# xingchensong/TouchNet

Hardware: AMD Instinct MI355X
Metric: audio+text tokens/sec/node (packed seq, full train step) + step MFU (higher is better)
Workload: dtype bf16

## Files before the change

touchnet_amd/csrc/gemm_kernel.h:

```cpp
#pragma once

#include <stdlib.h>

#include <type_traits>
#include <utility>
#include <vector>

#include "common.h"

namespace tn {
namespace gemm {

constexpr int BM = 256, BN = 256;
constexpr int SLOT = 32768;
constexpr int LDS_BYTES = 5 * SLOT;
constexpr int NT = 512;
constexpr int MAXSEG = 3;

typedef __attribute__((address_space(3))) void* lds_ptr_t;
typedef __attribute__((ext_vector_type(2))) uint32_t u32x2_t;
typedef __attribute__((ext_vector_type(4))) uint32_t u32x4_t;

struct Seg {
  const bf16_t* A;
  const bf16_t* B;
  long long lda, ldb;
  int K;
  int pad_;
};

struct Grp {
  bf16_t* C;
  long long ldc;
  int M, N, nbm, nbn;
  int start;
  int stages;
};

struct Rec {
  Seg seg;
  Grp grp;
  bf16_t* bias_out;
};
typedef const __attribute__((address_space(4))) Rec* rec_ptr_t;
constexpr int MAXTAB = 1024;
constexpr int TABCHUNK = 32;

constexpr int EPI_PLAIN = 0, EPI_GROUPED = 1, EPI_SWIGLU_FWD = 2, EPI_SWIGLU_BWD = 3, EPI_BIASG = 4, EPI_ROPE = 5;
constexpr int EPI_GELU_FWD = 6, EPI_GELU_BWD = 7, EPI_TABLE = 8;

struct Params {
  Seg seg[MAXSEG];
  int nseg;
  int M, N;
  bf16_t* C;
  bf16_t* Ct;
  const bf16_t* bias;
  long long ldc, ldct;
  int accumulate;
  const bf16_t* addend;
  long long ldadd;
  int nbm, nbn;
  int stages;
  int splitk, kchunk;
  float* ws;
  int tile0, ntiles;
  int c_f32;
  Grp grp[MAXSEG];
  int ngrp;
  bf16_t* C2;
  bf16_t* C3;
  const bf16_t* E1;
  const bf16_t* E2;
  long long lde;
  bf16_t* bias_out;
  float* bias_ws;
  const bf16_t* rope_cos;
  const bf16_t* rope_sin;
  int rope_d;
  const Rec* table;
};

__device__ __forceinline__ int xcd_chunk(int bid, int total) {
  const int xcd = bid & 7, local = bid >> 3;
  const int q = total >> 3, r = total & 7;
  return (xcd < r ? xcd * (q + 1) : r * (q + 1) + (xcd - r) * q) + local;
}

__device__ __forceinline__ void panel_group(int vid, int nbm, int nbn, int& tm, int& tn) {
  constexpr int GM = 8;
  const int per_group = GM * nbn;
  const int g = vid / per_group, w = vid - g * per_group;
  const int gm = min(GM, nbm - g * GM);
  tm = g * GM + w % gm;
  tn = w / gm;
}

__device__ __forceinline__ void tile_of_block(int bid, int nbm, int nbn, int& tm, int& tn) {
  panel_group(xcd_chunk(bid, nbm * nbn), nbm, nbn, tm, tn);
}

typedef f32x16_t Acc[4][2];

constexpr int kPieceB[4] = {0, 2, 4, 6}, kPieceA[4] = {14, 18, 22, 26};
static_assert(kPieceB[3] < kPieceA[0], "every B piece is issued before the first A piece");

template <bool IS_A> constexpr int piece_at(int pos) {
  for (int i = 0; i < 4; ++i)
    if ((IS_A ? kPieceA[i] : kPieceB[i]) == pos) return i;
  return -1;
}
constexpr int early_piece_count() {
  int n = 0;
  for (int i = 0; i < 4; ++i) n += (kPieceB[i] < 8) + (kPieceA[i] < 8);
  return n;
}

template <bool KMAJ, bool M16 = false>
struct Stream {
  __amdgpu_buffer_rsrc_t rs;
  int soff;
  int step;
  int left;
  int seg;
  int ld2;
  int voff[4];

  __device__ __forceinline__ void set_voff(int wave, int lane) {
    if constexpr (!KMAJ) {
#pragma unroll
      for (int q = 0; q < 4; ++q) {
        const int row = wave * 32 + q * 8 + (lane >> 3);
        voff[q] = row * ld2 + (((lane & 7) ^ ((row >> 1) & 7)) << 4);
      }
    } else {
#pragma unroll
      for (int q = 0; q < 4; ++q) {
        const int k = wave * 8 + q * 2 + (lane >> 5);
        const int u = lane & 31;
        const int ch = M16 ? ((u & 3) ^ (((k >> 3) & 1) << 1)) : (u & 3);
        voff[q] = k * ld2 + ((((u >> 2) ^ (k & 3)) << 6) | (ch << 4));
      }
    }
  }

  __device__ __forceinline__ void open(const bf16_t* X, long long ld, int K, int R, int origin, int wave, int lane) {
    ld2 = (int)(ld * 2);
    if constexpr (!KMAJ) {
      const long long bytes = max((long long)(R - origin) * ld2, 0LL);
      rs = __builtin_amdgcn_make_buffer_rsrc((void*)(X + (long long)origin * ld), 0, (int)min(bytes, 0x7fffffffLL),
                                             0x00020000);
      step = 128;
    } else {
      const long long bytes = ((long long)(K - 1) * ld + (R - origin)) * 2;
      rs = __builtin_amdgcn_make_buffer_rsrc((void*)(X + origin), 0, (int)min(bytes, 0x7fffffffLL), 0x00020000);
      step = 64 * ld2;
    }
    set_voff(wave, lane);
    soff = 0;
    left = (K + 63) >> 6;
  }
  __device__ __forceinline__ void kill(const void* any) {
    rs = __builtin_amdgcn_make_buffer_rsrc((void*)any, 0, 0, 0x00020000);
    soff = 0;
    step = 0;
    left = 0x7fffffff;
  }
};

template <bool KMAJ, int NB>
struct Frags {
  bf16x8_t v[NB];
  u32x2_t h[KMAJ ? NB : 1][2];
};

template <int OFF>
__device__ __forceinline__ u32x2_t ds_tr16(uint32_t addr) {
  u32x2_t r;
  asm volatile("ds_read_b64_tr_b16 %0, %1 offset:%2" : "=v"(r) : "v"(addr), "n"(OFF));
  return r;
}

template <bool AK, bool BK, bool HAS_CT, bool SPLITK = false, bool OUT_F32 = false, int EPI = EPI_PLAIN>
struct Kernel {
  static_assert(EPI == EPI_PLAIN || EPI == EPI_GROUPED || EPI == EPI_BIASG || EPI == EPI_TABLE,
                "Kernel: plain / grouped / bias-gradient epilogues (the fused ones are Kernel16's)");
  static constexpr bool MULTI = EPI == EPI_GROUPED || EPI == EPI_TABLE;
  static constexpr bool BIASG = EPI == EPI_BIASG || EPI == EPI_TABLE;
  static_assert(!MULTI || (!HAS_CT && !SPLITK), "grouped launch: whole tiles, no transposed copy");
  static_assert(!BIASG || (AK && BK && !HAS_CT), "bias gradient: weight-gradient mode");
  struct Out {
    bf16_t* C;
    long long ldc;
    int M, N;
  };
  template <bool KMAJ, int NB>
  struct Reader {
    int x[4];
    __device__ __forceinline__ Reader(int lane, int row0 ) {
      const int l31 = lane & 31, hi = lane >> 5;
      if constexpr (!KMAJ) {
        const int f = (l31 >> 1) & 7;
#pragma unroll
        for (int q = 0; q < 4; ++q) x[q] = (row0 + l31) * 128 + (((2 * q + hi) ^ f) << 4);
      } else {
        const int s4 = lane & 15, j = s4 >> 2, w = s4 & 3, half = (lane >> 4) & 1;
#pragma unroll
        for (int b = 0; b < 4; ++b)
          x[b] = (8 * hi + j) * 512 + half * 32 + w * 8 + ((((row0 >> 5) + (b < NB ? b : 0)) ^ j) << 6);
      }
    }
    template <int Q, int B>
    __device__ __forceinline__ void read(const char* smem, int sbase, Frags<KMAJ, NB>& f) const {
      if constexpr (!KMAJ) {
        f.v[B] = __builtin_bit_cast(bf16x8_t, *reinterpret_cast<const u32x4_t*>(smem + sbase + x[Q] + B * 4096));
      } else {
        const uint32_t a = (uint32_t)(size_t)(lds_ptr_t)smem + (uint32_t)(sbase + x[B]);
        f.h[B][0] = ds_tr16<(16 * Q) * 512>(a);
        f.h[B][1] = ds_tr16<(16 * Q + 4) * 512>(a);
      }
    }
  };

  static __device__ __forceinline__ void wait_frags(Frags<AK, 4>& a, Frags<BK, 2>& b) {
    if constexpr (AK && BK) {
      asm volatile("s_waitcnt lgkmcnt(0)"
                   : "+v"(a.h[0][0]), "+v"(a.h[0][1]), "+v"(a.h[1][0]), "+v"(a.h[1][1]), "+v"(a.h[2][0]), "+v"(a.h[2][1]),
                     "+v"(a.h[3][0]), "+v"(a.h[3][1]), "+v"(b.h[0][0]), "+v"(b.h[0][1]), "+v"(b.h[1][0]), "+v"(b.h[1][1]));
    } else if constexpr (AK) {
      asm volatile("s_waitcnt lgkmcnt(0)"
                   : "+v"(a.h[0][0]), "+v"(a.h[0][1]), "+v"(a.h[1][0]), "+v"(a.h[1][1]), "+v"(a.h[2][0]), "+v"(a.h[2][1]),
                     "+v"(a.h[3][0]), "+v"(a.h[3][1]));
    } else if constexpr (BK) {
      asm volatile("s_waitcnt lgkmcnt(0)" : "+v"(b.h[0][0]), "+v"(b.h[0][1]), "+v"(b.h[1][0]), "+v"(b.h[1][1]));
    }
    if constexpr (AK) {
#pragma unroll
      for (int i = 0; i < 4; ++i) {
        const u32x4_t t = {a.h[i][0].x, a.h[i][0].y, a.h[i][1].x, a.h[i][1].y};
        a.v[i] = __builtin_bit_cast(bf16x8_t, t);
      }
    }
    if constexpr (BK) {
#pragma unroll
      for (int j = 0; j < 2; ++j) {
        const u32x4_t t = {b.h[j][0].x, b.h[j][0].y, b.h[j][1].x, b.h[j][1].y};
        b.v[j] = __builtin_bit_cast(bf16x8_t, t);
      }
    }
  }

  static __device__ __forceinline__ void run(const Params& p, char* smem) { body(p, smem); }

  static __device__ __forceinline__ void body(const Params& p, char* smem) {
    const int tid = threadIdx.x;
    int lane = tid & 63;
    const int wave = __builtin_amdgcn_readfirstlane(tid >> 6);
    const int wr = wave >> 2, wc = wave & 3;

    const int bid = blockIdx.x, G = gridDim.x;
    const int tiles = p.ntiles;
    const int mine = ((SPLITK ? tiles * p.splitk : tiles) - bid + G - 1) / G;
    const rec_ptr_t tab = (rec_ptr_t)p.table;
    auto seg_of = [&](int g) {
      if constexpr (EPI == EPI_TABLE) {
        Seg s;
        s.A = tab[g].seg.A;
        s.B = tab[g].seg.B;
        s.lda = tab[g].seg.lda;
        s.ldb = tab[g].seg.ldb;
        s.K = tab[g].seg.K;
        s.pad_ = 0;
        return s;
      } else {
        return p.seg[g];
      }
    };
    auto grp_of = [&](int g) {
      if constexpr (EPI == EPI_TABLE) {
        Grp r;
        r.C = tab[g].grp.C;
        r.ldc = tab[g].grp.ldc;
        r.M = tab[g].grp.M;
        r.N = tab[g].grp.N;
        r.nbm = tab[g].grp.nbm;
        r.nbn = tab[g].grp.nbn;
        r.start = tab[g].grp.start;
        r.stages = tab[g].grp.stages;
        return r;
      } else {
        return p.grp[g];
      }
    };
    auto origin_g = [&](int k, int& m0, int& n0, int& g) {
      int tm, tn, u = bid + k * G;
      if constexpr (SPLITK) u -= (u / tiles) * tiles;
      u += p.tile0;
      g = 0;
      if constexpr (EPI == EPI_TABLE) {
        u = xcd_chunk(u, tiles);
        int hi = p.ngrp - 1;
        while (g < hi) {
          const int mid = (g + hi + 1) >> 1;
          if (tab[mid].grp.start <= u) g = mid;
          else hi = mid - 1;
        }
      } else if constexpr (EPI == EPI_GROUPED) {
        if (p.ngrp > 1 && u >= p.grp[1].start) g = 1;
        if (p.ngrp > 2 && u >= p.grp[2].start) g = 2;
      }
      if constexpr (EPI == EPI_TABLE) {
        const Grp r = grp_of(g);
        panel_group(u - r.start, r.nbm, r.nbn, tm, tn);
      } else if constexpr (EPI == EPI_GROUPED) {
        const Grp r = grp_of(g);
        tile_of_block(u - r.start, r.nbm, r.nbn, tm, tn);
      } else {
        tile_of_block(u, p.nbm, p.nbn, tm, tn);
      }
      m0 = tm * BM;
      n0 = tn * BN;
    };
    auto origin = [&](int k, int& m0, int& n0) {
      int g;
      origin_g(k, m0, n0, g);
    };
    auto split_of = [&](int k) { return (bid + k * G) / tiles; };

    Stream<AK> sA;
    Stream<BK> sB;
    int ka = 0, kb = 0;
    auto open_a = [&](int s) {
      int m0, n0;
      origin(ka, m0, n0);
      if constexpr (SPLITK) {
        const int k0 = split_of(ka) * p.kchunk * 64, klen = min(p.seg[0].K - k0, p.kchunk * 64);
        if (klen > 0) sA.open(p.seg[0].A + (AK ? (long long)k0 * p.seg[0].lda : (long long)k0), p.seg[0].lda, klen, p.M,
                              m0, wave, lane);
        else sA.kill(p.C);
        sA.left = p.kchunk;
      } else if constexpr (MULTI) {
        int g;
        origin_g(ka, m0, n0, g);
        const Seg sg = seg_of(g);
        sA.open(sg.A, sg.lda, sg.K, grp_of(g).M, m0, wave, lane);
      } else {
        sA.open(p.seg[s].A, p.seg[s].lda, p.seg[s].K, p.M, m0, wave, lane);
      }
      sA.seg = s;
    };
    auto open_b = [&](int s) {
      int m0, n0;
      origin(kb, m0, n0);
      if constexpr (SPLITK) {
        const int k0 = split_of(kb) * p.kchunk * 64, klen = min(p.seg[0].K - k0, p.kchunk * 64);
        if (klen > 0) sB.open(p.seg[0].B + (BK ? (long long)k0 * p.seg[0].ldb : (long long)k0), p.seg[0].ldb, klen, p.N,
                              n0, wave, lane);
        else sB.kill(p.C);
        sB.left = p.kchunk;
      } else if constexpr (MULTI) {
        int g;
        origin_g(kb, m0, n0, g);
        const Seg sg = seg_of(g);
        sB.open(sg.B, sg.ldb, sg.K, grp_of(g).N, n0, wave, lane);
      } else {
        sB.open(p.seg[s].B, p.seg[s].ldb, p.seg[s].K, p.N, n0, wave, lane);
      }
      sB.seg = s;
    };
    auto adv_a = [&]() {
      sA.soff += sA.step;
      if (--sA.left == 0) {
        if (sA.seg + 1 < p.nseg) open_a(sA.seg + 1);
        else if (++ka < mine) open_a(0);
        else sA.kill(p.C);
      }
    };
    auto adv_b = [&]() {
      sB.soff += sB.step;
      if (--sB.left == 0) {
        if (sB.seg + 1 < p.nseg) open_b(sB.seg + 1);
        else if (++kb < mine) open_b(0);
        else sB.kill(p.C);
      }
    };
    auto piece_a = [&](int slot, int q) {
      __builtin_amdgcn_raw_ptr_buffer_load_lds(sA.rs, (lds_ptr_t)(smem + slot * SLOT + wave * 4096 + q * 1024), 16,
                                               sA.voff[q], sA.soff, 0, 0);
    };
    auto piece_b = [&](int slot, int q) {
      __builtin_amdgcn_raw_ptr_buffer_load_lds(sB.rs, (lds_ptr_t)(smem + slot * SLOT + wave * 4096 + q * 1024), 16,
                                               sB.voff[q], sB.soff, 0, 0);
    };
    open_a(0);
    open_b(0);

    Reader<AK, 4> ra(lane, wr * 128);
    Reader<BK, 2> rb(lane, wc * 64);

    Acc acc;
    auto zero_acc = [&]() {
#pragma unroll
      for (int i = 0; i < 4; ++i)
#pragma unroll
        for (int j = 0; j < 2; ++j)
#pragma unroll
          for (int r = 0; r < 16; ++r) acc[i][j][r] = 0.f;
    };
    zero_acc();

    Frags<AK, 4> ae, ao;
    Frags<BK, 2> be, bo;

#define TN_PIN() __builtin_amdgcn_sched_barrier(0)
    auto read_frag = [&](auto QC, auto FC, int sa, int sb, Frags<AK, 4>& a, Frags<BK, 2>& b) {
      constexpr int Q = decltype(QC)::value, F = decltype(FC)::value;
      if constexpr (F < 2) rb.template read<Q, F>(smem, sb * SLOT, b);
      else ra.template read<Q, F - 2>(smem, sa * SLOT, a);
    };
    auto read_all = [&](auto QC, int sa, int sb, Frags<AK, 4>& a, Frags<BK, 2>& b) {
      read_frag(QC, std::integral_constant<int, 0>{}, sa, sb, a, b);
      read_frag(QC, std::integral_constant<int, 1>{}, sa, sb, a, b);
      read_frag(QC, std::integral_constant<int, 2>{}, sa, sb, a, b);
      read_frag(QC, std::integral_constant<int, 3>{}, sa, sb, a, b);
      read_frag(QC, std::integral_constant<int, 4>{}, sa, sb, a, b);
      read_frag(QC, std::integral_constant<int, 5>{}, sa, sb, a, b);
    };
    auto mma = [&](const Frags<AK, 4>& a, const Frags<BK, 2>& b, int i, int j) {
      acc[i][j] = __builtin_amdgcn_mfma_f32_32x32x16_bf16(b.v[j], a.v[i], acc[i][j], 0, 0, 0);
    };

    float bsum = 0.f;
    bool bias_on = false;
    auto bias_accum = [&](const Frags<AK, 4>& a) {
      auto add = [&](const bf16x8_t& v) {
        const u32x4_t w = __builtin_bit_cast(u32x4_t, v);
        bsum += ((__uint_as_float(w.x << 16) + __uint_as_float(w.x & 0xffff0000u)) +
                 (__uint_as_float(w.y << 16) + __uint_as_float(w.y & 0xffff0000u))) +
                ((__uint_as_float(w.z << 16) + __uint_as_float(w.z & 0xffff0000u)) +
                 (__uint_as_float(w.w << 16) + __uint_as_float(w.w & 0xffff0000u)));
      };
      if (wc == 0) add(a.v[0]);
      else if (wc == 1) add(a.v[1]);
      else if (wc == 2) add(a.v[2]);
      else add(a.v[3]);
    };

    auto quarter = [&](auto NQC, auto P0C, const Frags<AK, 4>& ca, const Frags<BK, 2>& cb, Frags<AK, 4>& na,
                       Frags<BK, 2>& nb, int nsa, int nsb, int dst_b, int dst_a) {
      constexpr int P0 = decltype(P0C)::value;
      if constexpr (BIASG) {
        if (bias_on) bias_accum(ca);
        TN_PIN();
      }
      auto step = [&](auto MC) {
        constexpr int m = decltype(MC)::value;
        mma(ca, cb, m >> 1, m & 1);
        TN_PIN();
        if constexpr (m < 6) {
          read_frag(NQC, std::integral_constant<int, m>{}, nsa, nsb, na, nb);
          TN_PIN();
        }
        constexpr int pb = P0 < 0 ? -1 : piece_at<false>(P0 + m);
        constexpr int pa = P0 < 0 ? -1 : piece_at<true>(P0 + m);
        if constexpr (pb >= 0) {
          piece_b(dst_b, pb);
          if constexpr (pb == 3) adv_b();
          TN_PIN();
        }
        if constexpr (pa >= 0) {
          piece_a(dst_a, pa);
          if constexpr (pa == 3) adv_a();
          TN_PIN();
        }
      };
      step(std::integral_constant<int, 0>{});
      step(std::integral_constant<int, 1>{});
      step(std::integral_constant<int, 2>{});
      step(std::integral_constant<int, 3>{});
      step(std::integral_constant<int, 4>{});
      step(std::integral_constant<int, 5>{});
      step(std::integral_constant<int, 6>{});
      step(std::integral_constant<int, 7>{});
    };
    auto early_pieces = [&](int dst_b, int dst_a) {
      auto one = [&](auto MC) {
        constexpr int m = decltype(MC)::value;
        constexpr int pb = piece_at<false>(m), pa = piece_at<true>(m);
        if constexpr (pb >= 0) {
          piece_b(dst_b, pb);
          if constexpr (pb == 3) adv_b();
        }
        if constexpr (pa >= 0) {
          piece_a(dst_a, pa);
          if constexpr (pa == 3) adv_a();
        }
      };
      one(std::integral_constant<int, 0>{});
      one(std::integral_constant<int, 1>{});
      one(std::integral_constant<int, 2>{});
      one(std::integral_constant<int, 3>{});
      one(std::integral_constant<int, 4>{});
      one(std::integral_constant<int, 5>{});
      one(std::integral_constant<int, 6>{});
      one(std::integral_constant<int, 7>{});
    };
    auto next = [](int s, int d) { s += d; return s >= 5 ? s - 5 : s; };
    using I0 = std::integral_constant<int, 0>;
    using I1 = std::integral_constant<int, 1>;
    using I2 = std::integral_constant<int, 2>;
    using I3 = std::integral_constant<int, 3>;
    using NONE = std::integral_constant<int, -1>;

#pragma unroll
    for (int q = 0; q < 4; ++q) piece_a(0, q);
    adv_a();
#pragma unroll
    for (int q = 0; q < 4; ++q) piece_b(1, q);
    adv_b();
#pragma unroll
    for (int q = 0; q < 4; ++q) piece_a(2, q);
    adv_a();
    early_pieces(3, 4);
    asm volatile("s_waitcnt vmcnt(%0)" ::"n"(4 + early_piece_count()) : "memory");
    __builtin_amdgcn_s_barrier();
    int sa = 0, sb = 1;
    int pa = 4, pb = 3;

    auto trip = [&](auto LASTC) {
      constexpr bool LAST = decltype(LASTC)::value;
      const int sa1 = next(sa, 2), sb1 = next(sb, 2);
      __builtin_amdgcn_s_setprio(1);
      quarter(I1{}, std::integral_constant<int, 8>{}, ae, be, ao, bo, sa, sb, pb, pa);
      wait_frags(ao, bo);
      TN_PIN();
      quarter(I2{}, std::integral_constant<int, 16>{}, ao, bo, ae, be, sa, sb, pb, pa);
      wait_frags(ae, be);
      TN_PIN();
      quarter(I3{}, std::integral_constant<int, 24>{}, ae, be, ao, bo, sa, sb, pb, pa);
      __builtin_amdgcn_s_setprio(0);
      wait_frags(ao, bo);
      __builtin_amdgcn_s_waitcnt(0xc07f);
      asm volatile("s_waitcnt vmcnt(4)" ::: "memory");
      __builtin_amdgcn_s_barrier();
      __builtin_amdgcn_s_setprio(1);
      if constexpr (!LAST) {
        quarter(I0{}, I0{}, ao, bo, ae, be, sa1, sb1, sa, sb);
        __builtin_amdgcn_s_setprio(0);
        wait_frags(ae, be);
        TN_PIN();
      } else {
        if constexpr (BIASG) {
          if (bias_on) bias_accum(ao);
        }
#pragma unroll
        for (int m = 0; m < 8; ++m) mma(ao, bo, m >> 1, m & 1);
        __builtin_amdgcn_s_setprio(0);
      }
      pb = sa;
      pa = sb;
      sa = sa1;
      sb = sb1;
    };

    const int np_all = SPLITK ? p.kchunk : p.stages;
    for (int kc = 0; kc < mine; ++kc) {
      int np = np_all;
      if constexpr (BIASG) {
        int m0_, n0_, g_;
        origin_g(kc, m0_, n0_, g_);
        bias_on = n0_ == 0;
        if constexpr (EPI == EPI_TABLE) bias_on = bias_on && tab[g_].bias_out != nullptr;
        bsum = 0.f;
      }
      if constexpr (MULTI) {
        int m0_, n0_, g_;
        origin_g(kc, m0_, n0_, g_);
        np = grp_of(g_).stages;
      }
      read_all(I0{}, sa, sb, ae, be);
      wait_frags(ae, be);
      TN_PIN();
      for (int t = 1; t < np; ++t) trip(std::false_type{});
      trip(std::true_type{});
      int m0, n0, grp;
      origin_g(kc, m0, n0, grp);
      if constexpr (BIASG) {
        if (bias_on) {
          const float tot = bsum + __shfl_xor(bsum, 32, 64);
          const int m = m0 + wr * 128 + wc * 32 + (lane & 31);
          if (lane < 32) {
            if constexpr (SPLITK) {
              p.bias_ws[(long long)split_of(kc) * (p.nbm * BM) + m] = tot;
            } else if constexpr (EPI == EPI_TABLE) {
              if (m < tab[grp].grp.M) tab[grp].bias_out[m] = f2bf(tot);
            } else if (m < p.M) {
              p.bias_out[m] = f2bf(tot);
            }
          }
        }
      }
      if constexpr (SPLITK) {
        const int u = bid + kc * G, sp = u / tiles;
        epilogue_ws(p, acc, sp * tiles + (u - sp * tiles), wr * 128, wc * 64, lane);
      } else if constexpr (OUT_F32) {
        if constexpr (MULTI) {
          const Grp r = grp_of(grp);
          const Out o = {r.C, r.ldc, r.M, r.N};
          epilogue_f32(p, o, acc, m0 + wr * 128, n0 + wc * 64, lane);
        } else {
          const Out o = {p.C, p.ldc, p.M, p.N};
          epilogue_f32(p, o, acc, m0 + wr * 128, n0 + wc * 64, lane);
        }
      } else if constexpr (MULTI) {
        const Grp r = grp_of(grp);
        const Out o = {r.C, r.ldc, r.M, r.N};
        epilogue(p, o, acc, smem + (wave < 4 ? pb : pa) * SLOT + (wave & 3) * 8192, m0 + wr * 128, n0 + wc * 64, lane);
      } else {
        const Out o = {p.C, p.ldc, p.M, p.N};
        epilogue(p, o, acc, smem + (wave < 4 ? pb : pa) * SLOT + (wave & 3) * 8192, m0 + wr * 128, n0 + wc * 64, lane);
      }
      zero_acc();
      __builtin_amdgcn_s_waitcnt(0xc07f);
      __builtin_amdgcn_s_barrier();
      asm volatile("" : "+v"(lane));
      ra = Reader<AK, 4>(lane, wr * 128);
      rb = Reader<BK, 2>(lane, wc * 64);
      sA.set_voff(wave, lane);
      sB.set_voff(wave, lane);
      early_pieces(pb, pa);
    }
  }

  static __device__ __forceinline__ void epilogue_f32(const Params& p, const Out& o, Acc& acc, int wm0, int wn0, int lane) {
    const int l31 = lane & 31, hi = lane >> 5;
    float* C = reinterpret_cast<float*>(o.C);
    const bool add = p.accumulate != 0;
#pragma unroll
    for (int i = 0; i < 4; ++i) {
      const int m = wm0 + i * 32 + l31;
#pragma unroll
      for (int j = 0; j < 2; ++j)
#pragma unroll
        for (int g = 0; g < 4; ++g) {
          const int n = wn0 + j * 32 + 8 * g + 4 * hi;
          if (m < o.M && n < o.N) {
            f32x4_t* dst = reinterpret_cast<f32x4_t*>(C + (long long)m * o.ldc + n);
            f32x4_t v = {acc[i][j][4 * g], acc[i][j][4 * g + 1], acc[i][j][4 * g + 2], acc[i][j][4 * g + 3]};
            if (add) v += *dst;
            *dst = v;
          }
        }
    }
  }

  static __device__ __forceinline__ void epilogue_ws(const Params& p, Acc& acc, int slab, int lm0, int ln0, int lane) {
    const int l31 = lane & 31, hi = lane >> 5;
    float* base = p.ws + (long long)slab * (BM * BN);
#pragma unroll
    for (int i = 0; i < 4; ++i) {
      const int m = lm0 + i * 32 + l31;
#pragma unroll
      for (int j = 0; j < 2; ++j)
#pragma unroll
        for (int g = 0; g < 4; ++g) {
          const int n = ln0 + j * 32 + 8 * g + 4 * hi;
          const f32x4_t v = {acc[i][j][4 * g], acc[i][j][4 * g + 1], acc[i][j][4 * g + 2], acc[i][j][4 * g + 3]};
          *reinterpret_cast<f32x4_t*>(base + m * BN + n) = v;
        }
    }
  }

  static __device__ __forceinline__ void epilogue(const Params& p, const Out& o, Acc& acc, char* park, int wm0, int wn0,
                                                  int lane) {
    const int l31 = lane & 31, hi = lane >> 5;
    float bias_v[2][4][4];
    if (p.bias != nullptr) {
#pragma unroll
      for (int j = 0; j < 2; ++j)
#pragma unroll
        for (int g = 0; g < 4; ++g) {
          const int n = min(wn0 + j * 32 + 8 * g + 4 * hi, o.N - 4);
          const uint2 w = *reinterpret_cast<const uint2*>(p.bias + n);
          bias_v[j][g][0] = __uint_as_float(w.x << 16);
          bias_v[j][g][1] = __uint_as_float(w.x & 0xffff0000u);
          bias_v[j][g][2] = __uint_as_float(w.y << 16);
          bias_v[j][g][3] = __uint_as_float(w.y & 0xffff0000u);
        }
    }
    const bool acc_c = p.accumulate != 0 || p.addend != nullptr;
#pragma unroll
    for (int half = 0; half < 2; ++half) {
#pragma unroll
      for (int ii = 0; ii < 2; ++ii) {
        const int i = half * 2 + ii;
        const int row = ii * 32 + l31;
#pragma unroll
        for (int j = 0; j < 2; ++j)
#pragma unroll
          for (int g = 0; g < 4; ++g) {
            float v[4];
#pragma unroll
            for (int e = 0; e < 4; ++e) v[e] = acc[i][j][4 * g + e] + (p.bias != nullptr ? bias_v[j][g][e] : 0.f);
            const int chunk = (j * 4 + g) ^ (row & 7);
            const u32x2_t pk = {pack2bf(v[0], v[1]), pack2bf(v[2], v[3])};
            *reinterpret_cast<u32x2_t*>(park + row * 128 + chunk * 16 + hi * 8) = pk;
          }
      }
      asm volatile("s_waitcnt lgkmcnt(0)" ::: "memory");
#pragma unroll 4
      for (int it = 0; it < 8; ++it) {
        const int row = it * 8 + (lane >> 3), c = lane & 7;
        const u32x4_t pv = *reinterpret_cast<const u32x4_t*>(park + row * 128 + ((c ^ (row & 7)) << 4));
        uint4 v = make_uint4(pv.x, pv.y, pv.z, pv.w);
        const int m = wm0 + half * 64 + row, n = wn0 + c * 8;
        if (m < o.M && n < o.N) {
          bf16_t* dst = o.C + (long long)m * o.ldc + n;
          if (acc_c) {
            Vec16<bf16_t> o, nw;
            o.load(p.addend != nullptr ? p.addend + (long long)m * p.ldadd + n : dst);
            nw.raw = v;
            float fo[8], fn[8];
            o.unpack(fo);
            nw.unpack(fn);
#pragma unroll
            for (int e = 0; e < 8; ++e) fn[e] += fo[e];
            nw.pack(fn);
            v = nw.raw;
          }
          *reinterpret_cast<uint4*>(dst) = v;
        }
      }
      if constexpr (HAS_CT) {
#pragma unroll 2
        for (int it = 0; it < 8; ++it) {
          const int n_l = it * 8 + (lane >> 3), mg = lane & 7;
          uint32_t w[4];
#pragma unroll
          for (int e2 = 0; e2 < 4; ++e2) {
            uint32_t lo, hi16;
            {
              const int row = mg * 8 + 2 * e2;
              lo = *reinterpret_cast<const uint16_t*>(park + row * 128 + ((((n_l >> 3) ^ (row & 7))) << 4) + (n_l & 7) * 2);
            }
            {
              const int row = mg * 8 + 2 * e2 + 1;
              hi16 = *reinterpret_cast<const uint16_t*>(park + row * 128 + ((((n_l >> 3) ^ (row & 7))) << 4) + (n_l & 7) * 2);
            }
            w[e2] = lo | (hi16 << 16);
          }
          const int n = wn0 + n_l, m = wm0 + half * 64 + mg * 8;
          if (n < o.N && m < o.M)
            *reinterpret_cast<uint4*>(p.Ct + (long long)n * p.ldct + m) = make_uint4(w[0], w[1], w[2], w[3]);
        }
      }
    }
  }
};

template <bool AK, bool BK, bool HAS_CT, bool SPLITK = false, bool OUT_F32 = false, int EPI = EPI_PLAIN>
__global__ __launch_bounds__(NT, 2) void gemm_kernel(const Params p) {
  __shared__ __attribute__((aligned(1024))) char smem[LDS_BYTES];
  Kernel<AK, BK, HAS_CT, SPLITK, OUT_F32, EPI>::run(p, smem);
}

}
}
```

Measured before the change: 23880.

## Spread bias-gradient row sums across MFMA steps using per-wave fragment permutation

In the bias-gradient GEMM variant, each wave's A-fragment reads are XOR-permuted by its column index, so the fragment it must sum for the bias is always slot 0. That removes the runtime branch on wc. The bf16 pair-sums are split into eight small pieces interleaved between the MFMA steps instead of one block at the start of each quarter. The epilogues undo the permutation when mapping accumulator rows to output rows. The bias sum is now computed unconditionally, with the bias_on check moved to the write, which adds a few VALU ops for tiles that don't need it.

```diff
diff --git a/touchnet_amd/csrc/gemm_kernel.h b/touchnet_amd/csrc/gemm_kernel.h
--- a/touchnet_amd/csrc/gemm_kernel.h
+++ b/touchnet_amd/csrc/gemm_kernel.h
@@ -197,7 +197,8 @@
   template <bool KMAJ, int NB>
   struct Reader {
     int x[4];
-    __device__ __forceinline__ Reader(int lane, int row0 ) {
+    __device__ __forceinline__ Reader(int lane, int row0 ,
+                                      int perm = 0) {
       const int l31 = lane & 31, hi = lane >> 5;
       if constexpr (!KMAJ) {
         const int f = (l31 >> 1) & 7;
@@ -207,7 +208,7 @@
         const int s4 = lane & 15, j = s4 >> 2, w = s4 & 3, half = (lane >> 4) & 1;
 #pragma unroll
         for (int b = 0; b < 4; ++b)
-          x[b] = (8 * hi + j) * 512 + half * 32 + w * 8 + ((((row0 >> 5) + (b < NB ? b : 0)) ^ j) << 6);
+          x[b] = (8 * hi + j) * 512 + half * 32 + w * 8 + ((((row0 >> 5) + (b < NB ? b ^ perm : 0)) ^ j) << 6);
       }
     }
     template <int Q, int B>
@@ -395,7 +396,8 @@
     open_a(0);
     open_b(0);
 
-    Reader<AK, 4> ra(lane, wr * 128);
+    const int aperm = BIASG ? wc : 0;
+    Reader<AK, 4> ra(lane, wr * 128, aperm);
     Reader<BK, 2> rb(lane, wc * 64);
 
     Acc acc;
@@ -430,33 +432,43 @@
       acc[i][j] = __builtin_amdgcn_mfma_f32_32x32x16_bf16(b.v[j], a.v[i], acc[i][j], 0, 0, 0);
     };
 
-    float bsum = 0.f;
-    bool bias_on = false;
+    float bsum = 0.f, bx = 0.f, by = 0.f, bz = 0.f;
+    auto bias_piece = [&](auto MC, const Frags<AK, 4>& a) {
+      constexpr int m = decltype(MC)::value;
+      const u32x4_t w = __builtin_bit_cast(u32x4_t, a.v[0]);
+      auto pair = [](uint32_t u) { return __uint_as_float(u << 16) + __uint_as_float(u & 0xffff0000u); };
+      auto here = [](float& v) { asm volatile("" : "+v"(v)); };
+      if constexpr (m == 0) here(bx = pair(w.x));
+      else if constexpr (m == 1) here(by = pair(w.y));
+      else if constexpr (m == 2) here(bx = bx + by);
+      else if constexpr (m == 3) here(bz = pair(w.z));
+      else if constexpr (m == 4) here(by = pair(w.w));
+      else if constexpr (m == 5) here(bz = bz + by);
+      else if constexpr (m == 6) here(bx = bx + bz);
+      else here(bsum += bx);
+    };
     auto bias_accum = [&](const Frags<AK, 4>& a) {
-      auto add = [&](const bf16x8_t& v) {
-        const u32x4_t w = __builtin_bit_cast(u32x4_t, v);
-        bsum += ((__uint_as_float(w.x << 16) + __uint_as_float(w.x & 0xffff0000u)) +
-                 (__uint_as_float(w.y << 16) + __uint_as_float(w.y & 0xffff0000u))) +
-                ((__uint_as_float(w.z << 16) + __uint_as_float(w.z & 0xffff0000u)) +
-                 (__uint_as_float(w.w << 16) + __uint_as_float(w.w & 0xffff0000u)));
-      };
-      if (wc == 0) add(a.v[0]);
-      else if (wc == 1) add(a.v[1]);
-      else if (wc == 2) add(a.v[2]);
-      else add(a.v[3]);
+      bias_piece(std::integral_constant<int, 0>{}, a);
+      bias_piece(std::integral_constant<int, 1>{}, a);
+      bias_piece(std::integral_constant<int, 2>{}, a);
+      bias_piece(std::integral_constant<int, 3>{}, a);
+      bias_piece(std::integral_constant<int, 4>{}, a);
+      bias_piece(std::integral_constant<int, 5>{}, a);
+      bias_piece(std::integral_constant<int, 6>{}, a);
+      bias_piece(std::integral_constant<int, 7>{}, a);
     };
 
     auto quarter = [&](auto NQC, auto P0C, const Frags<AK, 4>& ca, const Frags<BK, 2>& cb, Frags<AK, 4>& na,
                        Frags<BK, 2>& nb, int nsa, int nsb, int dst_b, int dst_a) {
       constexpr int P0 = decltype(P0C)::value;
-      if constexpr (BIASG) {
-        if (bias_on) bias_accum(ca);
-        TN_PIN();
-      }
       auto step = [&](auto MC) {
         constexpr int m = decltype(MC)::value;
         mma(ca, cb, m >> 1, m & 1);
         TN_PIN();
+        if constexpr (BIASG) {
+          bias_piece(MC, ca);
+          TN_PIN();
+        }
         if constexpr (m < 6) {
           read_frag(NQC, std::integral_constant<int, m>{}, nsa, nsb, na, nb);
           TN_PIN();
@@ -550,9 +562,7 @@
         wait_frags(ae, be);
         TN_PIN();
       } else {
-        if constexpr (BIASG) {
-          if (bias_on) bias_accum(ao);
-        }
+        if constexpr (BIASG) bias_accum(ao);
 #pragma unroll
         for (int m = 0; m < 8; ++m) mma(ao, bo, m >> 1, m & 1);
         __builtin_amdgcn_s_setprio(0);
@@ -566,13 +576,7 @@
     const int np_all = SPLITK ? p.kchunk : p.stages;
     for (int kc = 0; kc < mine; ++kc) {
       int np = np_all;
-      if constexpr (BIASG) {
-        int m0_, n0_, g_;
-        origin_g(kc, m0_, n0_, g_);
-        bias_on = n0_ == 0;
-        if constexpr (EPI == EPI_TABLE) bias_on = bias_on && tab[g_].bias_out != nullptr;
-        bsum = 0.f;
-      }
+      if constexpr (BIASG) bsum = 0.f;
       if constexpr (MULTI) {
         int m0_, n0_, g_;
         origin_g(kc, m0_, n0_, g_);
@@ -586,6 +590,8 @@
       int m0, n0, grp;
       origin_g(kc, m0, n0, grp);
       if constexpr (BIASG) {
+        bool bias_on = n0 == 0;
+        if constexpr (EPI == EPI_TABLE) bias_on = bias_on && tab[grp].bias_out != nullptr;
         if (bias_on) {
           const float tot = bsum + __shfl_xor(bsum, 32, 64);
           const int m = m0 + wr * 128 + wc * 32 + (lane & 31);
@@ -602,29 +608,31 @@
       }
       if constexpr (SPLITK) {
         const int u = bid + kc * G, sp = u / tiles;
-        epilogue_ws(p, acc, sp * tiles + (u - sp * tiles), wr * 128, wc * 64, lane);
+        epilogue_ws(p, acc, sp * tiles + (u - sp * tiles), wr * 128, wc * 64, lane, aperm);
       } else if constexpr (OUT_F32) {
         if constexpr (MULTI) {
           const Grp r = grp_of(grp);
           const Out o = {r.C, r.ldc, r.M, r.N};
-          epilogue_f32(p, o, acc, m0 + wr * 128, n0 + wc * 64, lane);
+          epilogue_f32(p, o, acc, m0 + wr * 128, n0 + wc * 64, lane, aperm);
         } else {
           const Out o = {p.C, p.ldc, p.M, p.N};
-          epilogue_f32(p, o, acc, m0 + wr * 128, n0 + wc * 64, lane);
+          epilogue_f32(p, o, acc, m0 + wr * 128, n0 + wc * 64, lane, aperm);
         }
       } else if constexpr (MULTI) {
         const Grp r = grp_of(grp);
         const Out o = {r.C, r.ldc, r.M, r.N};
-        epilogue(p, o, acc, smem + (wave < 4 ? pb : pa) * SLOT + (wave & 3) * 8192, m0 + wr * 128, n0 + wc * 64, lane);
+        epilogue(p, o, acc, smem + (wave < 4 ? pb : pa) * SLOT + (wave & 3) * 8192, m0 + wr * 128, n0 + wc * 64, lane,
+                 aperm);
       } else {
         const Out o = {p.C, p.ldc, p.M, p.N};
-        epilogue(p, o, acc, smem + (wave < 4 ? pb : pa) * SLOT + (wave & 3) * 8192, m0 + wr * 128, n0 + wc * 64, lane);
+        epilogue(p, o, acc, smem + (wave < 4 ? pb : pa) * SLOT + (wave & 3) * 8192, m0 + wr * 128, n0 + wc * 64, lane,
+                 aperm);
       }
       zero_acc();
       __builtin_amdgcn_s_waitcnt(0xc07f);
       __builtin_amdgcn_s_barrier();
       asm volatile("" : "+v"(lane));
-      ra = Reader<AK, 4>(lane, wr * 128);
+      ra = Reader<AK, 4>(lane, wr * 128, aperm);
       rb = Reader<BK, 2>(lane, wc * 64);
       sA.set_voff(wave, lane);
       sB.set_voff(wave, lane);
@@ -632,13 +640,14 @@
     }
   }
 
-  static __device__ __forceinline__ void epilogue_f32(const Params& p, const Out& o, Acc& acc, int wm0, int wn0, int lane) {
+  static __device__ __forceinline__ void epilogue_f32(const Params& p, const Out& o, Acc& acc, int wm0, int wn0, int lane,
+                                                      int perm) {
     const int l31 = lane & 31, hi = lane >> 5;
     float* C = reinterpret_cast<float*>(o.C);
     const bool add = p.accumulate != 0;
 #pragma unroll
     for (int i = 0; i < 4; ++i) {
-      const int m = wm0 + i * 32 + l31;
+      const int m = wm0 + (i ^ perm) * 32 + l31;
 #pragma unroll
       for (int j = 0; j < 2; ++j)
 #pragma unroll
@@ -654,12 +663,13 @@
     }
   }
 
-  static __device__ __forceinline__ void epilogue_ws(const Params& p, Acc& acc, int slab, int lm0, int ln0, int lane) {
+  static __device__ __forceinline__ void epilogue_ws(const Params& p, Acc& acc, int slab, int lm0, int ln0, int lane,
+                                                     int perm) {
     const int l31 = lane & 31, hi = lane >> 5;
     float* base = p.ws + (long long)slab * (BM * BN);
 #pragma unroll
     for (int i = 0; i < 4; ++i) {
-      const int m = lm0 + i * 32 + l31;
+      const int m = lm0 + (i ^ perm) * 32 + l31;
 #pragma unroll
       for (int j = 0; j < 2; ++j)
 #pragma unroll
@@ -672,7 +682,7 @@
   }
 
   static __device__ __forceinline__ void epilogue(const Params& p, const Out& o, Acc& acc, char* park, int wm0, int wn0,
-                                                  int lane) {
+                                                  int lane, int perm) {
     const int l31 = lane & 31, hi = lane >> 5;
     float bias_v[2][4][4];
     if (p.bias != nullptr) {
@@ -694,7 +704,7 @@
 #pragma unroll
       for (int ii = 0; ii < 2; ++ii) {
         const int i = half * 2 + ii;
-        const int row = ii * 32 + l31;
+        const int row = (ii ^ (perm & 1)) * 32 + l31;
 #pragma unroll
         for (int j = 0; j < 2; ++j)
 #pragma unroll
@@ -713,7 +723,7 @@
         const int row = it * 8 + (lane >> 3), c = lane & 7;
         const u32x4_t pv = *reinterpret_cast<const u32x4_t*>(park + row * 128 + ((c ^ (row & 7)) << 4));
         uint4 v = make_uint4(pv.x, pv.y, pv.z, pv.w);
-        const int m = wm0 + half * 64 + row, n = wn0 + c * 8;
+        const int m = wm0 + (half ^ (perm >> 1)) * 64 + row, n = wn0 + c * 8;
         if (m < o.M && n < o.N) {
           bf16_t* dst = o.C + (long long)m * o.ldc + n;
           if (acc_c) {
@@ -749,7 +759,7 @@
             }
             w[e2] = lo | (hi16 << 16);
           }
-          const int n = wn0 + n_l, m = wm0 + half * 64 + mg * 8;
+          const int n = wn0 + n_l, m = wm0 + (half ^ (perm >> 1)) * 64 + mg * 8;
           if (n < o.N && m < o.M)
             *reinterpret_cast<uint4*>(p.Ct + (long long)n * p.ldct + m) = make_uint4(w[0], w[1], w[2], w[3]);
         }
```

Result: no change. 24070, median of 6 (+0.8%).
